# dallison/subspace

Hardware: AMD Instinct MI355X
Metric: GiB/s CRC32 over batched payloads (device-resident); % of HBM3E read peak (higher is better)
Workload: dtype u8

## Files before the change

subspace_amd/_lib.py:

```python
from __future__ import annotations

import ctypes
import os
from pathlib import Path

_HERE = Path(__file__).resolve().parent
LIB_PATH = _HERE / "libsubspace_crc.so"
if os.environ.get("SUBSPACE_CRC_PROBE_LIB"):
    LIB_PATH = Path(os.environ["SUBSPACE_CRC_PROBE_LIB"])
DEV_LIB_PATH = _HERE / "libsubspace_crc_dev.so"
if os.environ.get("SUBSPACE_CRC_PROBE_DEV_LIB"):
    DEV_LIB_PATH = Path(os.environ["SUBSPACE_CRC_PROBE_DEV_LIB"])

EXPORTED_SYMBOLS = (
    "SubspaceCRC32",
    "SubspaceCRC32C",
    "subspace_crc_version",
    "subspace_crc_last_error",
    "subspace_crc_ctx_create",
    "subspace_crc_ctx_create_poly",
    "subspace_crc_ctx_destroy",
    "subspace_crc_ctx_check",
    "subspace_crc_ctx_reserve",
    "subspace_crc32_batch_uniform",
# ... 78 lines not shown
    u32, u64, vp, i32 = ctypes.c_uint32, ctypes.c_uint64, ctypes.c_void_p, ctypes.c_int
    lib.subspace_crc_testutil_fill_uniform.restype = i32
    lib.subspace_crc_testutil_fill_uniform.argtypes = [vp, u64, u64, u64, u64, u64, u64, vp]
    lib.subspace_crc_testutil_fill_ragged.restype = i32
    lib.subspace_crc_testutil_fill_ragged.argtypes = [vp, vp, vp, u64, u64, u64, u64, vp]
    lib.subspace_crc_testutil_tune.restype = i32
    lib.subspace_crc_testutil_tune.argtypes = [vp, i32, i32, i32]
    lib.subspace_crc_testutil_set.restype = i32
    lib.subspace_crc_testutil_set.argtypes = [vp, ctypes.c_char_p, i32]
    lib.subspace_crc_testutil_stream_read.restype = i32
    lib.subspace_crc_testutil_stream_read.argtypes = [vp, u64, vp, vp]
    lib.subspace_crc_testutil_stream_read_lds.restype = i32
    lib.subspace_crc_testutil_stream_read_lds.argtypes = [vp, u64, vp, ctypes.c_uint32, vp]
    lib.subspace_crc_testutil_uniform_alias.restype = i32
    lib.subspace_crc_testutil_uniform_alias.argtypes = [vp, vp, u64, vp, vp]
    lib.subspace_crc_testutil_probe.restype = i32
    lib.subspace_crc_testutil_probe.argtypes = [vp, vp]
    lib.subspace_crc_testutil_probe_waves.restype = u64
    lib.subspace_crc_testutil_probe_waves.argtypes = [vp, u64]
    lib.subspace_crc_testutil_slot_list_read.restype = i32
    lib.subspace_crc_testutil_slot_list_read.argtypes = [vp, u64, u32, u64, u32, vp, u64, vp]
    lib.subspace_crc_testutil_tile_list_read.restype = i32
    lib.subspace_crc_testutil_tile_list_read.argtypes = [vp, u64, vp, u64, vp]
    lib.subspace_crc_testutil_fault_words.restype = i32
    lib.subspace_crc_testutil_fault_words.argtypes = [vp, vp, vp]
    lib.subspace_crc_testutil_call_gen.restype = u32
    lib.subspace_crc_testutil_call_gen.argtypes = [vp]
    _dev = lib
    return lib


def last_error() -> str:
    msg = load().subspace_crc_last_error()
    return msg.decode() if msg else ""
```

subspace_amd/csrc/capi.hip:

```cpp
#include <hip/hip_runtime.h>

#include <algorithm>
#include <cstdarg>
#include <cstdio>
#include <cstring>
#include <mutex>
#include <vector>

#include "../../include/subspace_crc.h"
#include "crc_device.h"
#include "crc_math.h"
#include "ctx.h"

namespace subspace_amd {

template <int WG, bool SLOT, bool PROBE>
__global__ void crc32_uniform4k_kernel(const uint8_t*, u64, u64, const u32*, const u32*, u32, u32, u32*, int, u32*,
                                       SlotArgs);

struct TileDesc;
struct TileDesc8;
__global__ void crc32_ragged_count_desc_kernel(const u64*, u32, const u64*, u32, u64, u32, u32, u64*, u32*, u32*,
                                               u64*, u32*, u64, TileDesc8*, u32*, FaultRef);
__global__ void crc32_ragged_count_desc16_kernel(const u64*, u32, const u64*, u32, u64, u32, u32, u64*, u32*, u32*,
                                                 u64*, u32*, u64, TileDesc*, u32*, FaultRef);
__global__ void crc32_ragged_count_scan_kernel(const u64*, u32, const u64*, u32, u64, u32, u32, u64*, u32*, u32*,
                                               u64*, u32*, u32*, FaultRef);
__global__ void tile_segment_scan_kernel(const u32*, u32, u32, u32, const u64*, u64, u32*, u32*);
__global__ void segment_prefix_kernel(u32*, u64, u32, u32, const u64*, u64, u64*, u32*, FaultRef);
__global__ void crc32_ragged_desc_kernel(const u64*, u32, const u64*, u32, const u64*, u64, u64, TileDesc*, u32*,
                                         u64*, u64, u32*, FaultRef);
template <int WG>
__global__ void crc32_ragged_kernel(const uint8_t*, const u64*, u32, const u64*, u32, const u64*, u64,
                                    const TileDesc*, const u32*, const u32*, const u32*, HeadSeeds, u32*, u32*, u32,
                                    u64*, u64, u32*, FaultRef);
__global__ void crc32_ragged_final_kernel(const u64*, const u64*, u32, const u64*, u32, u64, const u32*, const u32*,
                                          u32, u32, u32*, const u32*, u32, u32*, u64*, u64, u32*, FaultRef);
__global__ void crc32_slot_finish_kernel(const u64*, uint8_t*, u64, const u64*, u64, u64, u64, int, int, u32,
                                         const u32*, const u32*, const u32*, u32*, u32*, u32*);
__global__ void slot_payload_offsets_kernel(u64, u64, u64, u64*, const u64*, u64, u64*);
__global__ void uniform_offsets_kernel(u64 stride, u64 length, u64 count, u64* offsets, u64* lengths);
template <int WG>
__global__ void crc32_long_kernel(const uint8_t*, u64, u32, u32, const u32*, const u32*, u32, u32, u32*, u32);
__global__ void crc32_long_final_kernel(const u32*, const u32*, u32, u32, u32, u32, u32*, u64*, u64, u32*);
template <int WG, bool SLOT, bool PROBE, int G>
__global__ void crc32_small_kernel(const u32*, const u32*, SmallArgs);

}

using namespace subspace_amd;

namespace {

thread_local char g_err[512] = "";

int fail(int code, const char* fmt, ...) {
  va_list ap;
  va_start(ap, fmt);
  vsnprintf(g_err, sizeof(g_err), fmt, ap);
  va_end(ap);
  return code;
}
int hip_fail(hipError_t e, const char* what) {
  return fail(SUBSPACE_CRC_EHIP, "%s: %s", what, hipGetErrorString(e));
}
#define HIP_TRY(call)                                   \
  do {                                                  \
    hipError_t e_ = (call);                             \
    if (e_ != hipSuccess) return hip_fail(e_, #call);   \
// ... 54 lines not shown
        c->ws_stream = c->ws_call_stream;
        c->ws_recorded = true;
      }
      c->ws_waited = false;
    }
  }
  CallScope(const CallScope&) = delete;
  CallScope& operator=(const CallScope&) = delete;
};

int use_workspace(subspace_crc_ctx* c, hipStream_t st) {
  if (c->ws_waited) return SUBSPACE_CRC_OK;
  if (!c->ws_done) HIP_TRY(hipEventCreateWithFlags(&c->ws_done, hipEventDisableTiming));
  if (c->ws_recorded && c->ws_stream != st && !capturing(st)) HIP_TRY(hipStreamWaitEvent(st, c->ws_done, 0));
  c->ws_waited = true;
  c->ws_call_stream = st;
  return SUBSPACE_CRC_OK;
}

const char* fault_text(u32 f) {
  if (f & kFaultTicket) return "a look-back scan ticket was beyond its grid (stale scan state)";
  if (f & kFaultLookbackSpin) return "a look-back scan predecessor never published (stale scan state)";
  if (f & kFaultSlotRing) return "a fused slot kernel finishing wave never received a payload CRC";
  return "unknown fault";
}

int fault_status(subspace_crc_ctx* c, hipStream_t st) {
  u32 f = 0;
  HIP_TRY(hipMemcpyAsync(&f, c->d_fault, sizeof(u32), hipMemcpyDeviceToHost, st));
  HIP_TRY(hipStreamSynchronize(st));
  if (f == 0) return SUBSPACE_CRC_OK;
  if (f & kFaultSlotRing) {
    HIP_TRY(hipDeviceSynchronize());
    HIP_TRY(hipMemcpy(&f, c->d_fault, sizeof(u32), hipMemcpyDeviceToHost));
    HIP_TRY(hipMemset(c->d_slot_counter, 0, kSlotCounters * kCountWords * sizeof(u64)));
    HIP_TRY(hipDeviceSynchronize());
  }
  HIP_TRY(hipMemsetAsync(c->d_fault, 0, sizeof(u32), st));
  HIP_TRY(hipStreamSynchronize(st));
  c->scan_dirty = true;
  return fail(SUBSPACE_CRC_EFAULT, "device fault 0x%x: %s; the results of the calls since the last check are not valid",
              f, fault_text(f));
}

struct TileGeom {
  u64 nw, nkmax, nwb, nseg, nblk;
};
TileGeom tile_geom(const subspace_crc_ctx* c, u64 tiles) {
  TileGeom g;
  g.nw = (u64)c->num_cus * (kRaggedWG / 64);
  g.nkmax = ceil_div(tiles ? tiles : 1, g.nw);
  g.nwb = ceil_div(g.nw, 64);
  g.nseg = g.nkmax * g.nwb;
  g.nblk = ceil_div(g.nkmax, 64) * g.nwb;
  return g;
// ... 209 lines not shown
        default: crc32_small_kernel<512, true, false, 32><<<blocks, 512, lds, st>>>(c->d_tab, c->d_laneops, a);
#undef SMALL_SLOT_CASE
      }
    }
  } else {
    a.zero_word = c->zero_word;
    c->zero_word = nullptr;
    switch (g) {
#define SMALL_CASE(G) \
  case G: crc32_small_kernel<512, false, false, G><<<blocks, 512, lds, st>>>(c->d_tab, c->d_laneops, a); break;
      SMALL_CASE(1) SMALL_CASE(2) SMALL_CASE(4) SMALL_CASE(8) SMALL_CASE(16)
      default: crc32_small_kernel<512, false, false, 32><<<blocks, 512, lds, st>>>(c->d_tab, c->d_laneops, a);
#undef SMALL_CASE
    }
  }
  HIP_TRY(hipGetLastError());
  return SUBSPACE_CRC_OK;
}

bool small_slot_fused(int32_t checksum_size, int32_t metadata_size) {
  return (u32)checksum_size <= kSlotFusedMaxMeta && (u32)metadata_size <= kSlotFusedMaxMeta;
}

int ensure_slot_ws(subspace_crc_ctx* c, u64 count) {
  if (count <= c->s_capacity) return SUBSPACE_CRC_OK;
  (void)hipFree(c->d_crc0);
  (void)hipFree(c->d_soff);
  (void)hipFree(c->d_slen);
  c->d_crc0 = nullptr;
  c->d_soff = nullptr;
  c->d_slen = nullptr;
  c->s_capacity = 0;
  HIP_TRY(hipMalloc(&c->d_crc0, count * sizeof(u32)));
  HIP_TRY(hipMalloc(&c->d_soff, count * sizeof(u64)));
  HIP_TRY(hipMalloc(&c->d_slen, count * sizeof(u64)));
  c->s_capacity = count;
  return SUBSPACE_CRC_OK;
}

int check_slot_args(int32_t checksum_size, int32_t metadata_size, uint32_t mode) {
  if (mode != SUBSPACE_CRC_SLOT_CALCULATE && mode != SUBSPACE_CRC_SLOT_VERIFY)
    return fail(SUBSPACE_CRC_EINVAL, "unknown slot mode %u", mode);
  if (checksum_size < 4) return fail(SUBSPACE_CRC_EINVAL, "checksum_size %d < 4", checksum_size);
  if (metadata_size < 0) return fail(SUBSPACE_CRC_EINVAL, "metadata_size %d < 0", metadata_size);
  return SUBSPACE_CRC_OK;
}
// ... 111 lines not shown
  if (e == hipSuccess) e = hipMemset(c->d_slot_counter, 0, kSlotCounters * kCountWords * sizeof(u64));
  if (e == hipSuccess) e = hipMalloc(&c->d_fault, 4 * sizeof(u32));
  if (e == hipSuccess) e = hipMemset(c->d_fault, 0, 4 * sizeof(u32));
  if (e == hipSuccess) e = hipEventCreateWithFlags(&c->ws_done, hipEventDisableTiming);
  if (e == hipSuccess) e = hipDeviceSynchronize();
  if (e == hipSuccess)
    e = hipFuncSetAttribute((const void*)crc32_ragged_kernel<kRaggedWG>, hipFuncAttributeMaxDynamicSharedMemorySize,
                            (int)ragged_lds_bytes());
  if (e == hipSuccess)
    e = hipFuncSetAttribute((const void*)crc32_long_kernel<kRaggedWG>, hipFuncAttributeMaxDynamicSharedMemorySize,
                            (int)ragged_lds_bytes());
  {
    const void* small_fns[] = {
        (const void*)crc32_small_kernel<512, false, false, 1>,  (const void*)crc32_small_kernel<512, true, false, 1>,
        (const void*)crc32_small_kernel<512, false, false, 2>,  (const void*)crc32_small_kernel<512, true, false, 2>,
        (const void*)crc32_small_kernel<512, false, false, 4>,  (const void*)crc32_small_kernel<512, true, false, 4>,
        (const void*)crc32_small_kernel<512, false, false, 8>,  (const void*)crc32_small_kernel<512, true, false, 8>,
        (const void*)crc32_small_kernel<512, false, false, 16>, (const void*)crc32_small_kernel<512, true, false, 16>,
        (const void*)crc32_small_kernel<512, false, false, 32>, (const void*)crc32_small_kernel<512, true, false, 32>};
    for (const void* f : small_fns)
      if (e == hipSuccess)
        e = hipFuncSetAttribute(f, hipFuncAttributeMaxDynamicSharedMemorySize, (int)small_lds_bytes() + 16);
  }
  if (e != hipSuccess) {
    subspace_crc_ctx_destroy(c);
    return hip_fail(e, "context setup");
  }
  *out = c;
  return SUBSPACE_CRC_OK;
}

void subspace_crc_ctx_destroy(subspace_crc_ctx* c) {
  if (!c) return;
  if (c->ws_done && c->ws_recorded) (void)hipEventSynchronize(c->ws_done);
  if (c->hcompute) (void)hipStreamSynchronize(c->hcompute);
  for (auto& h : c->hstage) {
    if (h.stream) (void)hipStreamSynchronize(h.stream);
    if (h.copied) (void)hipEventDestroy(h.copied);
    (void)hipFree(h.dbuf);
    (void)hipFree(h.dsizes);
    (void)hipFree(h.dres);
    (void)hipFree(h.derr);
    (void)hipHostFree(h.hres);
    (void)hipHostFree(h.herr);
    if (h.done) (void)hipEventDestroy(h.done);
    if (h.stream) (void)hipStreamDestroy(h.stream);
// ... 147 lines not shown

int subspace_crc32_slots(subspace_crc_ctx* c, const subspace_crc_slot* dev_slots, uint64_t count,
                         uint64_t max_message_size, int32_t checksum_size, int32_t metadata_size, uint32_t mode,
                         uint32_t* dev_status, uint32_t* dev_error_count, void* stream) {
  g_err[0] = 0;
  if (!c) return fail(SUBSPACE_CRC_EINVAL, "ctx is null");
  CallScope scope(c);
  int rc = check_slot_args(checksum_size, metadata_size, mode);
  if (rc) return rc;
  hipStream_t st = (hipStream_t)stream;
  if (count == 0) {
    if (dev_error_count) HIP_TRY(hipMemsetAsync(dev_error_count, 0, sizeof(u32), st));
    return SUBSPACE_CRC_OK;
  }
  if (!dev_slots) return fail(SUBSPACE_CRC_EINVAL, "null device pointer");
  if (count >= (1ull << 32)) return fail(SUBSPACE_CRC_EINVAL, "count %llu exceeds 2^32-1", (unsigned long long)count);
  HIP_TRY(hipSetDevice(c->device));
  const u64* rec = reinterpret_cast<const u64*>(dev_slots);
  const bool small = max_message_size <= kSmallMaxExt && c->small_path;
  if (small && small_slot_fused(checksum_size, metadata_size)) {
    const SmallSlot ss{rec, 3, 0, ~0ull, mode, checksum_size, metadata_size, dev_status, nullptr, dev_error_count};
    return small_run(c, nullptr, rec + 1, 3, rec + 2, 3, count, 0u, 0u, nullptr, st, &ss, small_lanes(max_message_size));
  }
  rc = use_workspace(c, st);
  if (rc) return rc;
  rc = ensure_slot_ws(c, count);
  if (rc) return rc;
  want_zeroed(c, dev_error_count);
  if (small) {
    rc = small_run(c, nullptr, rec + 1, 3, rec + 2, 3, count, 0u, 0u, c->d_crc0, st, nullptr,
                   small_lanes(max_message_size));
  } else {
    const u64 cap = count * ((max_message_size + 15 + 8191) / 8192) + 1;
    rc = ragged_run(c, nullptr, cap, rec + 1, 3, rec + 2, 3, count, 0u, 0u, c->d_crc0, st, 0);
  }
  const bool zeroed = was_zeroed(c, dev_error_count);
  if (rc) return rc;
  return slot_finish(c, rec, nullptr, 0, nullptr, 0, count, ~0ull, checksum_size, metadata_size, mode, dev_status,
                     dev_error_count, st, nullptr, zeroed);
}

}

namespace {

int slots_strided_impl(subspace_crc_ctx* c, void* dev_buffer, uint64_t slot_stride, uint64_t count,
// ... 340 lines not shown
```

subspace_amd/csrc/crc_combine.hip:

```cpp
#include "crc_desc.h"

namespace subspace_amd {

constexpr int kScanThreads = 256;
constexpr int kScanItems = (int)(kScanTile / kScanThreads);
static_assert(kScanTile % kScanThreads == 0, "segment-prefix scan: whole items per thread");
constexpr int kCountItems = (int)(kCountTile / kScanThreads);
static_assert(kCountTile % kScanThreads == 0, "tile-count scan: whole items per thread");
constexpr u64 kFlagAggregate = 1, kFlagInclusive = 2;

struct SumOp {
  using T = u64;
  static __device__ __forceinline__ T identity() { return 0; }
  static __device__ __forceinline__ T op(T a, T b) { return a + b; }
  static __device__ __forceinline__ u64 pack(u64 flag, T v) { return (flag << 62) | v; }
  static __device__ __forceinline__ u64 flag(u64 s) { return s >> 62; }
  static __device__ __forceinline__ T value(u64 s) { return s & ((1ull << 62) - 1); }
};

struct XorOp {
  using T = u32;
  static __device__ __forceinline__ T identity() { return 0; }
  static __device__ __forceinline__ T op(T a, T b) { return a ^ b; }
  static __device__ __forceinline__ u64 pack(u64 flag, T v) { return (flag << 32) | v; }
// ... 146 lines not shown
  for (int j = 0; j < kCountItems; j++) {
    const u64 i = base + (u64)(j * kScanThreads + tid);
    if (i <= count) tile_base[i] = sx[j * kScanThreads + tid];
  }
}

constexpr int kFusedThreads = 1024;
constexpr int kFusedItems = (int)(kCountTile / kFusedThreads);
static_assert(kCountTile % kFusedThreads == 0, "fused scan: whole items per thread");
template <bool WIDE>
__device__ __forceinline__ void count_desc_body(const u64* __restrict__ offsets, u32 ostride,
                                                const u64* __restrict__ lengths, u32 lstride, u64 count, u32 init,
                                                u32 final_xor, u64* __restrict__ tile_base, u32* __restrict__ out,
                                                u32* __restrict__ zero_word, u64* __restrict__ status,
                                                u32* __restrict__ ticket, u64 capacity, void* __restrict__ desc,
                                                u32* __restrict__ overflow, FaultRef fault) {
  __shared__ u64 sx[kCountTile];
  __shared__ u32 sw[WIDE ? 1 : kFusedThreads / 64][kDesc8WaveWords][64];
  bool stale;
  const u64 tile = scan_ticket(ticket, fault, &stale, true);
  if (stale) return;
  const u64 base = tile * kCountTile;
  const int tid = threadIdx.x;
  if (WIDE && tid == 0) overflow[1] = 1u;
  u64 so[kFusedItems], L[kFusedItems], nt[kFusedItems];
  bool bad = false;
#pragma unroll
  for (int j = 0; j < kFusedItems; j++) {
    const u64 i = base + (u64)(j * kFusedThreads + tid);
    so[j] = L[j] = nt[j] = 0;
    if (i < count) {
      so[j] = offsets[i * ostride];
      L[j] = lengths[i * lstride];
      nt[j] = msg_tiles(so[j], L[j]);
      out[i] = nt[j] == 0 ? init ^ final_xor : 0u;
      if (!WIDE && nt[j] &&
          ((((so[j] & ~(u64)15) + ((nt[j] - 1) << 13)) >> kDesc8StartBits) | ((nt[j] - 1) >> kDesc8AfterBits)))
        bad = true;
    } else if (i == count && zero_word) {
      *zero_word = 0u;
    }
    sx[j * kFusedThreads + tid] = nt[j];
  }
  if (bad) overflow[2] = 1u;
  __syncthreads();
  u64 x[kFusedItems];
#pragma unroll
// ... 122 lines not shown
```

subspace_amd/csrc/crc_device.h:

```cpp
#pragma once
#include <hip/hip_runtime.h>
#include <stdint.h>

namespace subspace_amd {

using u32 = uint32_t;
using u64 = uint64_t;
using i64 = int64_t;
using u32x4 = __attribute__((ext_vector_type(4))) unsigned int;
using u32x2 = __attribute__((ext_vector_type(2))) unsigned int;

constexpr u32 kLdsTables = 0;
constexpr u32 kLdsOps = 128u * 1024u;

constexpr int kLaneOpWords = 8 * 16 * 32;
constexpr int kUniSlotOpZ4096 = kLaneOpWords * 4 / 512;
constexpr int kUniSlotOpZ64 = kUniSlotOpZ4096 + 1;
constexpr int kUniOpSlots = kUniSlotOpZ64 + 4;
constexpr int kUniOpSlotsOneChain = kUniSlotOpZ4096 + 1;
constexpr u32 kUniRing = kLdsOps + kUniOpSlots * 512u;
constexpr int uni_ring_results(int waves) { return kUniRing + (u32)waves * 1024u <= 160u * 1024u ? 256 : 128; }
constexpr size_t uniform_lds_bytes(int waves) { return kUniRing + (size_t)waves * 4u * uni_ring_results(waves); }
static_assert(uniform_lds_bytes(16) <= 160u * 1024u && uniform_lds_bytes(8) <= 160u * 1024u,
              "uniform kernel LDS exceeds 160 KiB");
// ... 2 lines not shown
constexpr int kSlotFinishers = 4;
constexpr u32 kSlotRingBytesPerWave = 2u * 8u * kSlotRingRounds;
constexpr u32 uniform_slot_mism_word(int waves) { return kUniSlotRing + (u32)waves * kSlotRingBytesPerWave; }
constexpr size_t uniform_slot_lds_bytes(int waves) { return uniform_slot_mism_word(waves) + 16u; }
static_assert(uniform_slot_lds_bytes(8) <= 160u * 1024u, "slot kernel LDS exceeds 160 KiB");

struct SlotArgs {
  u64 prefix_size;
  u32 mode;
  u32* status;
  u32* crc_out;
  u32* error_count;
  u64* counter;
  u64* probe;
  u32* fault;
  u32 checksum_size;
  u32 metadata_size;
};
constexpr u32 kSlotFusedMaxMeta = 64;

constexpr u32 kFaultLookbackSpin = 1u;
constexpr u32 kFaultTicket = 2u;
constexpr u32 kFaultSlotRing = 4u;
__device__ __forceinline__ void raise_fault(u32* fault, u32 bit) {
  if (fault) __hip_atomic_fetch_or(fault, bit, __ATOMIC_RELAXED, __HIP_MEMORY_SCOPE_AGENT);
}
struct FaultRef {
  u32* word;
  u32 gen;
};
__device__ __forceinline__ void raise_scan_fault(FaultRef f, u32 bit) {
  if (f.word) {
    __hip_atomic_fetch_or(f.word, bit, __ATOMIC_RELAXED, __HIP_MEMORY_SCOPE_AGENT);
    __hip_atomic_store(f.word + 1, f.gen, __ATOMIC_RELAXED, __HIP_MEMORY_SCOPE_AGENT);
  }
}
__device__ __forceinline__ bool scan_faulted(FaultRef f) {
  return f.word && f.word[1] == f.gen;
}
constexpr u32 kSpinBound = 1u << 20;
constexpr int kProbeWords = 8;

constexpr int kNumTileOps = 21;
constexpr int kRagOpZ4096 = kLaneOpWords * 4 / 512;
constexpr int kRagOpZTile = kRagOpZ4096 + 1;
constexpr int kRagZ64Words = kLaneOpWords + (1 + kNumTileOps) * 128;
constexpr int kRagLdsOpWords = kRagZ64Words + 512;
constexpr int kRagHighOps = kRagLdsOpWords;
constexpr int kNumInvOps = 13;
constexpr int kRagInvOps = kRagHighOps + (31 - kNumTileOps) * 128;
constexpr int kRagNibInvOps = kRagInvOps + kNumInvOps * 128;
constexpr int kNumNibInvOps = 45;
constexpr int kRagOpWords = kRagNibInvOps + kNumNibInvOps * 128;
constexpr size_t ragged_lds_bytes() { return kLdsOps + (size_t)kRagLdsOpWords * 4u; }
static_assert(ragged_lds_bytes() <= 160u * 1024u, "ragged kernel LDS exceeds 160 KiB");

constexpr int kSmallOpInv = kUniOpSlots;
constexpr int kSmallInvOps = 12;
constexpr int kSmallOpSlots = kSmallOpInv + kSmallInvOps;
constexpr int kSmallOpZC = kSmallOpSlots;
constexpr int kSmallLaneOpSlots = kSmallOpZC + 5;
constexpr u32 kSmallMaxExt = 4096;
constexpr u32 kSmallRing = kLdsOps + (u32)(kSmallOpSlots + 1) * 512u;
constexpr u32 kSmallRingTiles = 32;
constexpr u32 kSmallRingBytesPerWave = kSmallRingTiles * 2u * 8u;
constexpr u32 kRp2Entries = 256;
constexpr u32 kRp2MaxTiles = kRp2Entries * 32u / 64u;
constexpr u32 kRp2EntS = kSmallRing;
constexpr u32 kRp2EntM = kRp2EntS + 8u * kRp2Entries;
constexpr u32 kRp2Ring = kRp2EntM + 4u * kRp2Entries;
constexpr u32 kRp2Starts = kRp2Ring + 8u * kRp2Entries;
constexpr u32 kRp2First = kRp2Starts + 8u * kRp2MaxTiles;
constexpr u32 kRp2Misc = kRp2First + 4u * kRp2MaxTiles;
constexpr u32 kRp2Counts = kRp2Misc + 176u;
constexpr u32 kRp2Bytes = kRp2Counts + 128u - kSmallRing;
constexpr u32 kSmallShared = 8u * kSmallRingBytesPerWave > kRp2Bytes ? 8u * kSmallRingBytesPerWave : kRp2Bytes;
constexpr size_t small_lds_bytes() { return kSmallRing + kSmallShared; }
static_assert(small_lds_bytes() + 16u <= 160u * 1024u, "small-message kernel LDS (+ mismatch word) exceeds 160 KiB");
// ... 248 lines not shown
  if constexpr (SUBSPACE_ISSUE_PRIO > 0) __builtin_amdgcn_s_setprio(0);
}

__device__ __forceinline__ u64 tilecrc_index(u64 w, u64 k, u32 nwb) {
  return ((((k >> 6) * nwb + (w >> 6)) << 6 | (w & 63)) << 6) | (k & 63);
}
__device__ __forceinline__ u64 local_index(u64 w, u64 k, u32 nwb) {
  return ((((k >> 6) * nwb + (w >> 6)) << 6 | (k & 63)) << 6) | (w & 63);
}
__device__ __forceinline__ u32 tile_prefix(const u32* __restrict__ local, const u32* __restrict__ segx, u32 nw,
                                           u32 nwb, u64 tau) {
  const u32 t = (u32)tau, k = t / nw, w = t - k * nw;
  return segx[(u64)k * nwb + (w >> 6)] ^ local[local_index(w, k, nwb)];
}

__device__ __forceinline__ void reset_scan_state(u64* status, u64 nwords, u32* ticket) {
  const u64 g = (u64)blockIdx.x * blockDim.x + threadIdx.x, stride = (u64)gridDim.x * blockDim.x;
  for (u64 i = g; i < nwords; i += stride) __hip_atomic_store(&status[i], 0ull, __ATOMIC_RELAXED, __HIP_MEMORY_SCOPE_AGENT);
  if (g == 0) __hip_atomic_store(ticket, 0u, __ATOMIC_RELAXED, __HIP_MEMORY_SCOPE_AGENT);
}

#ifndef SUBSPACE_COUNT_GROUPS
#define SUBSPACE_COUNT_GROUPS 1
#endif
constexpr u32 kCountGroups = SUBSPACE_COUNT_GROUPS;
constexpr u32 kCountWords = 16;
__device__ __forceinline__ void add_call_mismatches(u64* counter, u32 n, u32* error_count) {
  if constexpr (kCountGroups == 1) {
    const u64 old = atomicAdd(reinterpret_cast<unsigned long long*>(counter), (1ull << 32) | (u64)n);
    if ((u32)(old >> 32) == gridDim.x - 1u) {
      *error_count = (u32)old + n;
      __hip_atomic_store(counter, 0ull, __ATOMIC_RELAXED, __HIP_MEMORY_SCOPE_AGENT);
    }
    return;
  }
  const u32 G = gridDim.x, g = blockIdx.x % kCountGroups;
  const u32 ng = (G - g + kCountGroups - 1u) / kCountGroups;
  const u64 old = atomicAdd(reinterpret_cast<unsigned long long*>(counter + 1 + g), (1ull << 32) | (u64)n);
  if ((u32)(old >> 32) == ng - 1u) {
    const u32 tot = (u32)old + n;
    __hip_atomic_store(counter + 1 + g, 0ull, __ATOMIC_RELAXED, __HIP_MEMORY_SCOPE_AGENT);
    const u32 groups = G < kCountGroups ? G : kCountGroups;
    const u64 o2 = atomicAdd(reinterpret_cast<unsigned long long*>(counter), (1ull << 32) | (u64)tot);
    if ((u32)(o2 >> 32) == groups - 1u) {
      *error_count = (u32)o2 + tot;
      __hip_atomic_store(counter, 0ull, __ATOMIC_RELAXED, __HIP_MEMORY_SCOPE_AGENT);
    }
  }
}
// ... 9 lines not shown
```

subspace_amd/csrc/ctx.h:

```cpp
#pragma once
#include <hip/hip_runtime.h>

#include <mutex>

#include "../../include/subspace_crc.h"
#include "crc_device.h"
#include "crc_math.h"

namespace subspace_amd {

struct DevHooks {
  u64* probe = nullptr;
  hipError_t (*uniform)(bool slot, unsigned blocks, hipStream_t st, const uint8_t* base, u64 stride, u64 count,
                        const u32* tab, const u32* ops, u32 init, u32 final_xor, u32* out, u32* zero_word,
                        SlotArgs sa) = nullptr;
  hipError_t (*small_slot)(unsigned blocks, size_t lds, hipStream_t st, const u32* tab, const u32* ops,
                           const SmallArgs& a) = nullptr;
};

constexpr uint32_t kCtxMagic = 0x43524353u;

}

struct subspace_crc_ctx {
// ... 34 lines not shown
    hipEvent_t copied = nullptr;
    hipEvent_t done = nullptr;
    uint8_t* dbuf = nullptr;
    subspace_amd::u64* dsizes = nullptr;
    subspace_amd::u32* dres = nullptr;
    subspace_amd::u32* derr = nullptr;
    subspace_amd::u32* hres = nullptr;
    subspace_amd::u32* herr = nullptr;
  } hstage[2];
  subspace_amd::u64 h_bytes = 0, h_slots = 0;
  subspace_crc_slot* l_hrec = nullptr;
  subspace_crc_slot* l_drec = nullptr;
  subspace_amd::u32* l_dstatus = nullptr;
  subspace_amd::u32* l_hstatus = nullptr;
  subspace_amd::u64 l_capacity = 0;
  subspace_amd::u32* d_crc0 = nullptr;
  subspace_amd::u64* d_soff = nullptr;
  subspace_amd::u64* d_slen = nullptr;
  subspace_amd::u64 s_capacity = 0;
  subspace_amd::u64* d_slot_counter = nullptr;
  subspace_amd::u32 slot_counter_next = 0;
  bool fused_slots = true;
  bool small_path = true;
  subspace_amd::DevHooks dev;
  subspace_amd::u32* d_fault = nullptr;
  subspace_amd::u32 call_gen = 0;
  std::recursive_mutex mu;
  int depth = 0;
  hipEvent_t ws_done = nullptr;
  hipStream_t ws_stream = nullptr;
  bool ws_recorded = false;
  bool ws_waited = false;
  hipStream_t ws_call_stream = nullptr;
};
```

subspace_amd/csrc/devtools.hip:

```cpp
#define SUBSPACE_DEV_TU 1
#include "crc_small.hip"
#include "crc_uniform.hip"
#include "ctx.h"

#include <algorithm>
#include <cstring>

namespace subspace_amd {
template __global__ void crc32_small_kernel<512, true, true, 32>(const u32*, const u32*, SmallArgs);
template __global__ void crc32_uniform4k_kernel<512, false, true>(const uint8_t*, u64, u64, const u32*, const u32*, u32,
                                                                  u32, u32*, int, u32*, SlotArgs);
template __global__ void crc32_uniform4k_kernel<512, true, true>(const uint8_t*, u64, u64, const u32*, const u32*, u32,
                                                                 u32, u32*, int, u32*, SlotArgs);
template __global__ void crc32_uniform4k_kernel<512, false, false>(const uint8_t*, u64, u64, const u32*, const u32*,
                                                                   u32, u32, u32*, int, u32*, SlotArgs);
}

using namespace subspace_amd;

namespace {

bool ctx_ok(const subspace_crc_ctx* c) {
  return c && c->magic == kCtxMagic && c->layout_bytes == (uint32_t)sizeof(subspace_crc_ctx);
}
// ... 39 lines not shown
  }();
  return e;
}

}

extern "C" {

int subspace_crc_testutil_set(subspace_crc_ctx* c, const char* key, int value) {
  if (!ctx_ok(c) || !key) return SUBSPACE_CRC_EINVAL;
  std::lock_guard<std::recursive_mutex> lk(c->mu);
  if (!std::strcmp(key, "stale_ticket")) {
    if (!c->d_scan_state) return SUBSPACE_CRC_EINVAL;
    const u32 v = (u32)value;
    if (hipSetDevice(c->device) != hipSuccess || hipDeviceSynchronize() != hipSuccess ||
        hipMemcpy(c->d_scan_state, &v, sizeof(u32), hipMemcpyHostToDevice) != hipSuccess)
      return SUBSPACE_CRC_EHIP;
    return SUBSPACE_CRC_OK;
  }
  bool* knob = !std::strcmp(key, "long_path")     ? &c->long_path
               : !std::strcmp(key, "fused_slots") ? &c->fused_slots
               : !std::strcmp(key, "fused_prep")  ? &c->fused_prep
               : !std::strcmp(key, "small_path")  ? &c->small_path
                                                  : nullptr;
  if (!knob) return SUBSPACE_CRC_EINVAL;
  *knob = value != 0;
  return SUBSPACE_CRC_OK;
}

int subspace_crc_testutil_tune(subspace_crc_ctx* c, int uniform_wg, int uniform_blocks, int uniform_order) {
  if (!ctx_ok(c) || uniform_wg != 512 || uniform_order < 0 || uniform_order > 3 || uniform_blocks < 0)
    return SUBSPACE_CRC_EINVAL;
  std::lock_guard<std::recursive_mutex> lk(c->mu);
  c->uniform_blocks = uniform_blocks;
  c->uniform_order = uniform_order;
  return SUBSPACE_CRC_OK;
}

int subspace_crc_testutil_probe(subspace_crc_ctx* c, void* dev_words) {
  if (!ctx_ok(c)) return SUBSPACE_CRC_EINVAL;
  std::lock_guard<std::recursive_mutex> lk(c->mu);
  if (dev_words) {
    if (hipSetDevice(c->device) != hipSuccess || set_lds_attributes() != hipSuccess) return SUBSPACE_CRC_EHIP;
    c->dev.uniform = uniform_probe;
    c->dev.small_slot = small_slot_probe;
  }
// ... 35 lines not shown
```

subspace_amd/csrc/testutil.hip:

```cpp
#include <hip/hip_runtime.h>
#include <stdint.h>

#include "crc_device.h"

namespace {

__device__ __forceinline__ uint64_t splitmix64(uint64_t x) {
  uint64_t z = x + 0x9E3779B97F4A7C15ull;
  z = (z ^ (z >> 30)) * 0xBF58476D1CE4E5B9ull;
  z = (z ^ (z >> 27)) * 0x94D049BB133111EBull;
  return z ^ (z >> 31);
}

__global__ void synth_fill_kernel(uint8_t* __restrict__ base, const uint64_t* __restrict__ offsets,
                                  const uint64_t* __restrict__ lengths, uint64_t stride, uint64_t length,
                                  uint64_t count, uint64_t first_id, uint64_t id_stride, uint64_t seed) {
  for (uint64_t m = blockIdx.x; m < count; m += gridDim.x) {
    const uint64_t off = offsets ? offsets[m] : m * stride;
    const uint64_t len = lengths ? lengths[m] : length;
    const uint64_t id = first_id + m * id_stride;
    const uint64_t key = seed ^ (id << 32);
    uint8_t* dst = base + off;
    const uint64_t units = (len + 7) >> 3;
    const bool aligned8 = (off & 7) == 0;
// ... 219 lines not shown
  };
  u64 a0, a1;
  u32 n0, n1;
  desc(0, a0, n0);
  u32x4 A[8], B[8];
  load(A, a0, n0);
  u64 k = 0;
  for (; k + 1 < nk; k += 2) {
    desc(k + 1, a1, n1);
    drain_before_issue();
    load(B, a1, n1);
    fold(A);
    desc(k + 2, a0, n0);
    drain_before_issue();
    load(A, a0, n0);
    fold(B);
  }
  drain_before_issue();
  if (k < nk) fold(A);
  if (acc == 0x12345678u && ntiles == 1) lds_unused3[threadIdx.x] = acc;
  out[blockIdx.x * 512 + threadIdx.x] = acc;
}

}

extern "C" {

int subspace_crc_testutil_tile_list_read(const void* dev_tiles, uint64_t ntiles, unsigned* dev_out,
                                         uint64_t out_words, void* stream) {
  if (!dev_tiles || !dev_out || ntiles == 0) return -1;
  int dev = 0, cus = 0;
  if (hipGetDevice(&dev) != hipSuccess || hipDeviceGetAttribute(&cus, hipDeviceAttributeMultiprocessorCount, dev) != hipSuccess)
    return -2;
  if (out_words < (uint64_t)cus * 512) return -1;
  const size_t ldsb = subspace_amd::ragged_lds_bytes();
  if (hipFuncSetAttribute((const void*)tile_list_read_kernel, hipFuncAttributeMaxDynamicSharedMemorySize, (int)ldsb) !=
      hipSuccess)
    return -2;
  tile_list_read_kernel<<<(unsigned)cus, 512, ldsb, (hipStream_t)stream>>>(static_cast<const uint64_t*>(dev_tiles),
                                                                             ntiles, dev_out);
  return hipGetLastError() == hipSuccess ? 0 : -2;
}

int subspace_crc_testutil_slot_list_read(const void* dev_records, uint64_t count, uint32_t mode, uint64_t stride,
                                         uint32_t lds, unsigned* dev_out, uint64_t out_words, void* stream) {
  if (!dev_records || !dev_out || count == 0 || mode > 6) return -1;
  int dev = 0, cus = 0;
  if (hipGetDevice(&dev) != hipSuccess || hipDeviceGetAttribute(&cus, hipDeviceAttributeMultiprocessorCount, dev) != hipSuccess)
    return -2;
// ... 69 lines not shown
```

subspace_amd/gpu.py:

```python
from __future__ import annotations

import ctypes

from . import _lib

FINALIZE = 0x1
POLY_IEEE = 0xEDB88320
POLY_CASTAGNOLI = 0x82F63B78

SLOT_CALCULATE = 0
SLOT_VERIFY = 1
SLOT_OK, SLOT_MISMATCH, SLOT_UNCHECKED, SLOT_OVERSIZE = 0, 1, 2, 4
EFAULT = -5


class CrcError(RuntimeError):
    def __init__(self, msg: str, code: int = 0):
        super().__init__(msg)
        self.code = code


def _check(rc: int, what: str) -> None:
    if rc != 0:
        raise CrcError(f"{what} failed ({rc}): {_lib.last_error()}", rc)
# ... 145 lines not shown
def fill_uniform(buf, stride: int, length: int, count: int, *, seed: int, first_id: int = 0, id_stride: int = 1,
                 stream=None) -> None:
    _check(_lib.load_dev().subspace_crc_testutil_fill_uniform(
        _ptr(buf), stride, length, count, first_id, id_stride, seed, _stream_ptr(stream)), "fill_uniform")


def fill_ragged(buf, offsets, lengths, *, seed: int, first_id: int = 0, id_stride: int = 1, stream=None) -> None:
    _check(_lib.load_dev().subspace_crc_testutil_fill_ragged(
        _ptr(buf), _ptr(offsets), _ptr(lengths), int(offsets.numel()), first_id, id_stride, seed,
        _stream_ptr(stream)), "fill_ragged")


def slot_list_read(records, count: int, out, mode: int = 4, stride: int = 0, lds: bool = True, stream=None) -> None:
    _check(_lib.load_dev().subspace_crc_testutil_slot_list_read(
        _ptr(records), int(count), int(mode), int(stride), 1 if lds else 0, _ptr(out), int(out.numel()),
        _stream_ptr(stream)), "slot_list_read")


def tile_list_read(tiles, out, stream=None) -> None:
    _check(_lib.load_dev().subspace_crc_testutil_tile_list_read(
        _ptr(tiles), int(tiles.shape[0]), _ptr(out), int(out.numel()), _stream_ptr(stream)), "tile_list_read")


def stream_read(buf, out, stream=None) -> None:
    if int(out.numel()) < 256 * 512:
        raise ValueError("out needs 131072 words")
    _check(_lib.load_dev().subspace_crc_testutil_stream_read(
        _ptr(buf), int(buf.numel() * buf.element_size()), _ptr(out), _stream_ptr(stream)), "stream_read")
```

Measured before the change: 5584.

## Add fused single-pass medium-message slot-list CRC kernel with per-wave message streaming

Adds a new kernel for slot lists whose messages fall between the small-path limit and 32 KiB. Each wave streams whole messages in 8 KiB tiles with double-buffered loads, drawn from workgroup-level chunk tickets. It then folds the header/metadata CRC and writes or verifies the checksum in batches of 64, replacing the multi-kernel workspace path. This targets launch and workspace overheads and intermediate global traffic. The cost is a new spin-wait chunk ring with a fault path, plus a memory-read test utility.

```diff
diff --git a/subspace_amd/_lib.py b/subspace_amd/_lib.py
--- a/subspace_amd/_lib.py
+++ b/subspace_amd/_lib.py
@@ -124,6 +124,9 @@
     lib.subspace_crc_testutil_slot_list_read.argtypes = [vp, u64, u32, u64, u32, vp, u64, vp]
     lib.subspace_crc_testutil_tile_list_read.restype = i32
     lib.subspace_crc_testutil_tile_list_read.argtypes = [vp, u64, vp, u64, vp]
+    if hasattr(lib, "subspace_crc_testutil_msg_list_read"):
+        lib.subspace_crc_testutil_msg_list_read.restype = i32
+        lib.subspace_crc_testutil_msg_list_read.argtypes = [vp, u64, vp, u64, vp]
     lib.subspace_crc_testutil_fault_words.restype = i32
     lib.subspace_crc_testutil_fault_words.argtypes = [vp, vp, vp]
     lib.subspace_crc_testutil_call_gen.restype = u32
diff --git a/subspace_amd/csrc/capi.hip b/subspace_amd/csrc/capi.hip
--- a/subspace_amd/csrc/capi.hip
+++ b/subspace_amd/csrc/capi.hip
@@ -45,6 +45,8 @@
 __global__ void crc32_long_final_kernel(const u32*, const u32*, u32, u32, u32, u32, u32*, u64*, u64, u32*);
 template <int WG, bool SLOT, bool PROBE, int G>
 __global__ void crc32_small_kernel(const u32*, const u32*, SmallArgs);
+template <int WG>
+__global__ void crc32_medium_slots_kernel(const u32*, const u32*, MediumArgs);
 
 }
 
@@ -145,6 +147,7 @@
   if (f & kFaultTicket) return "a look-back scan ticket was beyond its grid (stale scan state)";
   if (f & kFaultLookbackSpin) return "a look-back scan predecessor never published (stale scan state)";
   if (f & kFaultSlotRing) return "a fused slot kernel finishing wave never received a payload CRC";
+  if (f & kFaultMediumChunk) return "a medium slot kernel wave never received its workgroup's next chunk";
   return "unknown fault";
 }
 
@@ -153,7 +156,7 @@
   HIP_TRY(hipMemcpyAsync(&f, c->d_fault, sizeof(u32), hipMemcpyDeviceToHost, st));
   HIP_TRY(hipStreamSynchronize(st));
   if (f == 0) return SUBSPACE_CRC_OK;
-  if (f & kFaultSlotRing) {
+  if (f & (kFaultSlotRing | kFaultMediumChunk)) {
     HIP_TRY(hipDeviceSynchronize());
     HIP_TRY(hipMemcpy(&f, c->d_fault, sizeof(u32), hipMemcpyDeviceToHost));
     HIP_TRY(hipMemset(c->d_slot_counter, 0, kSlotCounters * kCountWords * sizeof(u64)));
@@ -409,6 +412,28 @@
   return (u32)checksum_size <= kSlotFusedMaxMeta && (u32)metadata_size <= kSlotFusedMaxMeta;
 }
 
+bool medium_slot_list(const subspace_crc_ctx* c, u64 max_message_size, int32_t checksum_size, int32_t metadata_size) {
+  return c->medium_path && max_message_size > kSmallMaxExt && max_message_size <= kMedMaxMessage &&
+         small_slot_fused(checksum_size, metadata_size);
+}
+int medium_run(subspace_crc_ctx* c, const u64* rec, u64 count, int32_t checksum_size, int32_t metadata_size, u32 mode,
+               u32* status, u32* error_count, hipStream_t st) {
+  MediumArgs a{};
+  a.rec = rec;
+  a.count = count;
+  a.mode = mode;
+  a.checksum_size = (u32)checksum_size;
+  a.metadata_size = (u32)metadata_size;
+  a.status = status;
+  a.error_count = error_count;
+  a.counter = c->d_slot_counter + kCountWords * (c->slot_counter_next++ % kSlotCounters);
+  a.fault = c->d_fault;
+  const unsigned blocks = (unsigned)grid_for(c, ceil_div(count, kMedChunk), 1);
+  crc32_medium_slots_kernel<512><<<blocks, 512, medium_lds_bytes(), st>>>(c->d_tab, c->d_rops, a);
+  HIP_TRY(hipGetLastError());
+  return SUBSPACE_CRC_OK;
+}
+
 int ensure_slot_ws(subspace_crc_ctx* c, u64 count) {
   if (count <= c->s_capacity) return SUBSPACE_CRC_OK;
   (void)hipFree(c->d_crc0);
@@ -566,6 +591,9 @@
       if (e == hipSuccess)
         e = hipFuncSetAttribute(f, hipFuncAttributeMaxDynamicSharedMemorySize, (int)small_lds_bytes() + 16);
   }
+  if (e == hipSuccess)
+    e = hipFuncSetAttribute((const void*)crc32_medium_slots_kernel<512>, hipFuncAttributeMaxDynamicSharedMemorySize,
+                            (int)medium_lds_bytes());
   if (e != hipSuccess) {
     subspace_crc_ctx_destroy(c);
     return hip_fail(e, "context setup");
@@ -759,6 +787,8 @@
     const SmallSlot ss{rec, 3, 0, ~0ull, mode, checksum_size, metadata_size, dev_status, nullptr, dev_error_count};
     return small_run(c, nullptr, rec + 1, 3, rec + 2, 3, count, 0u, 0u, nullptr, st, &ss, small_lanes(max_message_size));
   }
+  if (medium_slot_list(c, max_message_size, checksum_size, metadata_size))
+    return medium_run(c, rec, count, checksum_size, metadata_size, mode, dev_status, dev_error_count, st);
   rc = use_workspace(c, st);
   if (rc) return rc;
   rc = ensure_slot_ws(c, count);
diff --git a/subspace_amd/csrc/crc_combine.hip b/subspace_amd/csrc/crc_combine.hip
--- a/subspace_amd/csrc/crc_combine.hip
+++ b/subspace_amd/csrc/crc_combine.hip
@@ -192,7 +192,7 @@
   if (stale) return;
   const u64 base = tile * kCountTile;
   const int tid = threadIdx.x;
-  if (WIDE && tid == 0) overflow[1] = 1u;
+  if (tid == 0) overflow[1] = WIDE ? 1u : 0u;
   u64 so[kFusedItems], L[kFusedItems], nt[kFusedItems];
   bool bad = false;
 #pragma unroll
diff --git a/subspace_amd/csrc/crc_device.h b/subspace_amd/csrc/crc_device.h
--- a/subspace_amd/csrc/crc_device.h
+++ b/subspace_amd/csrc/crc_device.h
@@ -48,6 +48,7 @@
 constexpr u32 kFaultLookbackSpin = 1u;
 constexpr u32 kFaultTicket = 2u;
 constexpr u32 kFaultSlotRing = 4u;
+constexpr u32 kFaultMediumChunk = 8u;
 __device__ __forceinline__ void raise_fault(u32* fault, u32 bit) {
   if (fault) __hip_atomic_fetch_or(fault, bit, __ATOMIC_RELAXED, __HIP_MEMORY_SCOPE_AGENT);
 }
@@ -80,6 +81,28 @@
 constexpr int kRagOpWords = kRagNibInvOps + kNumNibInvOps * 128;
 constexpr size_t ragged_lds_bytes() { return kLdsOps + (size_t)kRagLdsOpWords * 4u; }
 static_assert(ragged_lds_bytes() <= 160u * 1024u, "ragged kernel LDS exceeds 160 KiB");
+
+constexpr int kMedTileOps = 3;
+constexpr int kMedFillSlots = kRagOpZTile + kMedTileOps;
+constexpr int kMedOpZ64 = kMedFillSlots;
+constexpr int kMedOpInv = kMedOpZ64 + 4;
+constexpr int kMedOpSlots = kMedOpInv + kNumInvOps;
+constexpr u32 kMedCtl = kLdsOps + 512u * (u32)kMedOpSlots;
+constexpr u32 kMedRing = 16;
+constexpr size_t medium_lds_bytes() { return kMedCtl + 64u + 8u * kMedRing; }
+static_assert(medium_lds_bytes() <= 160u * 1024u, "medium slot kernel LDS exceeds 160 KiB");
+constexpr u32 kMedChunk = 16;
+constexpr u32 kMedMaxMessage = 32768;
+
+struct MediumArgs {
+  const u64* rec;
+  u64 count;
+  u32 mode, checksum_size, metadata_size;
+  u32* status;
+  u32* error_count;
+  u64* counter;
+  u32* fault;
+};
 
 constexpr int kSmallOpInv = kUniOpSlots;
 constexpr int kSmallInvOps = 12;
@@ -374,9 +397,13 @@
 
 #ifndef SUBSPACE_COUNT_GROUPS
 #define SUBSPACE_COUNT_GROUPS 1
+#elif !defined(SUBSPACE_AB_BUILD)
+#error "SUBSPACE_COUNT_GROUPS is a timing-only knob: build with tools/ab_lib.sh (SUBSPACE_AB_BUILD)"
 #endif
 constexpr u32 kCountGroups = SUBSPACE_COUNT_GROUPS;
 constexpr u32 kCountWords = 16;
+static_assert(kCountGroups >= 1 && kCountGroups + 1 <= kCountWords, "the group words overrun the counter entry");
+static_assert(kCountGroups + 2 <= kCountWords, "the group words reach the chunk ticket");
 __device__ __forceinline__ void add_call_mismatches(u64* counter, u32 n, u32* error_count) {
   if constexpr (kCountGroups == 1) {
     const u64 old = atomicAdd(reinterpret_cast<unsigned long long*>(counter), (1ull << 32) | (u64)n);
diff --git a/subspace_amd/csrc/crc_medium.hip b/subspace_amd/csrc/crc_medium.hip
--- /dev/null
+++ b/subspace_amd/csrc/crc_medium.hip
@@ -0,0 +1,325 @@
+#include "crc_device.h"
+
+namespace subspace_amd {
+
+namespace {
+constexpr u32 kMedHasChecksum = 4u;
+constexpr u32 kMedNone = 0xFFFFFFFFu;
+
+typedef __attribute__((address_space(1))) u64 glb_u64_t;
+typedef __attribute__((address_space(1))) u32 glb_u32_t;
+
+__device__ __forceinline__ u64 readlane64(u64 v, int l) {
+  const u32 lo = (u32)__builtin_amdgcn_readlane((int)(u32)v, l);
+  const u32 hi = (u32)__builtin_amdgcn_readlane((int)(u32)(v >> 32), l);
+  return ((u64)hi << 32) | lo;
+}
+
+struct MedMsg {
+  u64 s0;
+  u64 ext;
+  u64 pfx;
+  u64 len;
+  u64 nt;
+  u32 mis;
+  u32 idx;
+};
+
+template <int WG>
+struct MedOpFill {
+  static constexpr int kWords = (4 + kNumInvOps) * 128;
+  static constexpr int kIters = (kWords + WG - 1) / WG;
+  u32 v[kIters];
+  __device__ __forceinline__ void load(const u32* __restrict__ gops) {
+#pragma unroll
+    for (int i = 0; i < kIters; i++) {
+      const int t = min((int)threadIdx.x + i * WG, kWords - 1);
+      v[i] = gops[t < 512 ? kRagZ64Words + t : kRagInvOps + (t - 512)];
+    }
+  }
+  __device__ __forceinline__ void store(u32 sbase) const {
+#pragma unroll
+    for (int i = 0; i < kIters; i++) {
+      const int t = (int)threadIdx.x + i * WG;
+      if (t < kWords) lds_st(sbase + kLdsOps + 512u * (u32)kMedOpZ64 + 4u * (u32)t, v[i]);
+    }
+#pragma unroll
+    for (int i = 0; i < kIters; i++) asm volatile("" ::"v"(v[i]));
+  }
+};
+}
+
+template <int WG>
+__global__ __launch_bounds__(WG) void crc32_medium_slots_kernel(const u32* __restrict__ gtab,
+                                                                const u32* __restrict__ gops, MediumArgs a) {
+  extern __shared__ __attribute__((aligned(16))) u32 smem[];
+  const u32 sbase = (u32)(uintptr_t)smem;
+  const int lane = threadIdx.x & 63;
+  const u32 lc0 = sbase + ((u32)(lane & 31) << 2);
+  const u32 lc1 = lc0 + 0x10000u;
+  const u32 z64 = sbase + kLdsOps + 512u * (u32)kMedOpZ64 + 4u * (u32)(lane & 3);
+  const u32 lop = sbase + kLdsOps + 4u * (u32)(31 - (lane & 31));
+  const u32 ctl = sbase + kMedCtl, ring = ctl + 64u;
+  const bool calc = a.mode == 0u;
+  u32* const gticket = reinterpret_cast<u32*>(a.counter + (kCountWords - 1));
+  const u32 G = rfl(gridDim.x);
+
+  if (threadIdx.x == 0) {
+    lds_st(ctl, 0u);
+    lds_st(ctl + 8u, 0u);
+  }
+  if (threadIdx.x < kMedRing)
+    lds_st64(ring + 8u * threadIdx.x, threadIdx.x == 0 ? (u64)blockIdx.x : ~0ull);
+  __syncthreads();
+
+  LdsFill<WG, kMedFillSlots> fill;
+  fill.load(gtab, gops);
+  MedOpFill<WG> xfill;
+  xfill.load(gops);
+
+  auto draw = [&]() __attribute__((always_inline)) -> u32 {
+    u32 t = 0;
+    if (lane == 0)
+      t = __hip_atomic_fetch_add(reinterpret_cast<lds_u32_t*>((uintptr_t)ctl), 1u, __ATOMIC_RELAXED,
+                                 __HIP_MEMORY_SCOPE_WORKGROUP);
+    t = rfl(t);
+    const u32 q = t / kMedChunk, r = t % kMedChunk;
+    if (r == 0u) {
+      u32 g = 0;
+      if (lane == 0) g = atomicAdd(gticket, 1u);
+      if (lane == 0) lds_st64(ring + 8u * ((q + 1u) % kMedRing), (u64)(G + g) | ((u64)(q + 1u) << 32));
+    }
+    u64 e = 0;
+    u32 spins = 0;
+    for (;;) {
+      const u64 v = lds_ld64(ring + 8u * (q % kMedRing));
+      e = rfl64((u32)v, (u32)(v >> 32));
+      if ((u32)(e >> 32) == q) break;
+      if (++spins > kSpinBound) {
+        if (lane == 0) raise_fault(a.fault, kFaultMediumChunk);
+        return kMedNone;
+      }
+      __builtin_amdgcn_s_sleep(1);
+    }
+    const u64 idx = (u64)(u32)e * kMedChunk + r;
+    return idx < a.count ? (u32)idx : kMedNone;
+  };
+  auto rec_load = [&](u32 idx) __attribute__((always_inline)) -> u64 {
+    const u64* p = a.rec + 3ull * (idx == kMedNone ? 0u : idx) + (u32)min(lane, 2);
+    const u64 v = *p;
+    asm volatile("" ::"v"(p));
+    return v;
+  };
+  auto unpack = [&](u64 R, u32 idx) __attribute__((always_inline)) -> MedMsg {
+    MedMsg m;
+    m.pfx = readlane64(R, 0);
+    const u64 s = readlane64(R, 1);
+    m.len = idx == kMedNone ? 0ull : readlane64(R, 2);
+    m.idx = idx;
+    m.mis = (u32)s & 15u;
+    m.s0 = s & ~(u64)15;
+    m.ext = m.len ? m.len + m.mis : 0ull;
+    const u64 nt = (m.ext + 8191u) >> 13;
+    m.nt = nt ? nt : 1ull;
+    return m;
+  };
+  const u32 vo = (u32)lane * 128u;
+  auto load_line = [&](const MedMsg& m, u64 j, u32x4 (&L)[8]) __attribute__((always_inline)) {
+    const u64 rest = m.ext - (j << 13);
+    const u32 len = rest < 8192u ? (u32)rest : 8192u;
+    const u32 nrec = (len + 15u) & ~15u;
+    const auto r = __builtin_amdgcn_make_buffer_rsrc(reinterpret_cast<uint8_t*>(m.s0 + (j << 13)), (short)0,
+                                                     (int)nrec, kBufferRsrcFlags);
+#pragma unroll
+    for (int b = 0; b < 8; b++) L[b] = __builtin_amdgcn_raw_buffer_load_b128(r, vo + 16u * b, 0, 0);
+    __builtin_amdgcn_sched_barrier(0);
+  };
+
+  auto tile_value = [&](const u32x4 (&cur)[8], const MedMsg& m, u64 j) __attribute__((always_inline)) -> u32 {
+    const u64 rest = m.ext - (j << 13);
+    const u32 len = rest < 8192u ? (u32)rest : 8192u;
+    u32x4 d[8];
+#pragma unroll
+    for (int b = 0; b < 8; b++) d[b] = cur[b];
+    const bool head = j == 0 && m.mis != 0u, tail = len < 8192u && (len & 15u) != 0u;
+    if (head || tail) {
+      const int v0 = (int)len - 128 * lane;
+      const u32 hi = v0 <= 0 ? 0u : (v0 >= 128 ? 128u : (u32)v0);
+      const u32 lo = (head && lane == 0) ? m.mis : 0u;
+      keep_bytes(d, lo, hi);
+    }
+    const u32 crc = line_crc32_2chain(d, 0u, lc0, lc1, z64);
+    u32 v = lane_shift(lop, crc);
+    v ^= (u32)__builtin_amdgcn_update_dpp(0, (int)v, 0x111, 0xF, 0xF, false);
+    v ^= (u32)__builtin_amdgcn_update_dpp(0, (int)v, 0x112, 0xF, 0xF, false);
+    v ^= (u32)__builtin_amdgcn_update_dpp(0, (int)v, 0x114, 0xF, 0xF, false);
+    v ^= (u32)__builtin_amdgcn_update_dpp(0, (int)v, 0x118, 0xF, 0xF, false);
+    v ^= (u32)__builtin_amdgcn_update_dpp(0, (int)v, 0x142, 0xA, 0xF, false);
+    const u32 h0 = (u32)__builtin_amdgcn_readlane((int)v, 31), h1 = (u32)__builtin_amdgcn_readlane((int)v, 63);
+    return opmul(sbase, kRagOpZ4096, h0) ^ h1;
+  };
+
+  auto inv_bits = [&](u32 x, u32 bits, int nb) __attribute__((always_inline)) {
+    for (int b = 0; b < nb && __any(bits != 0u); b++) {
+      if (__any((bits & 1u) != 0u)) {
+        const u32 xm = opmul(sbase, kMedOpInv + b, x);
+        x = (bits & 1u) ? xm : x;
+      }
+      bits >>= 1;
+    }
+    return x;
+  };
+
+  u64 PFX = 0, PLEN = 0;
+  u32 PMIS = 0, PIDX = 0, PVAL = 0;
+  u32 mism = 0;
+
+  auto flush = [&](u32 n) __attribute__((always_inline)) {
+    const bool valid = (u32)lane < n;
+    const u64 pa = valid ? PFX : readlane64(PFX, 0);
+    const u64 L = valid ? PLEN : 0ull;
+    const u32 mis = valid ? PMIS : 0u;
+    u32 w[14];
+    {
+      const glb_u64_t* q = reinterpret_cast<const glb_u64_t*>(pa);
+#pragma unroll
+      for (int i = 0; i < 7; i++) {
+        const u64 x = q[i];
+        w[2 * i] = (u32)x;
+        w[2 * i + 1] = (u32)(x >> 32);
+      }
+      asm volatile("" ::"v"(q));
+    }
+    const bool has = (w[8] & kMedHasChecksum) != 0u;
+    const u32 F = calc ? (w[8] | kMedHasChecksum) : w[8];
+    const u32 S = w[12];
+    w[8] = F;
+    u32 h = 0xFFFFFFFFu;
+#pragma unroll
+    for (int i = 1; i < 12; i++) h = step4(h ^ w[i], lc0, lc1);
+    if (a.metadata_size) {
+      constexpr u32 kW = kSlotFusedMaxMeta / 4 + 2;
+      const u32 o1 = 48u + a.checksum_size, sh = o1 & 3u, ms = a.metadata_size;
+      const u32 nwords = (sh + ms + 3u) >> 2;
+      const glb_u32_t* p1 = reinterpret_cast<const glb_u32_t*>(pa + (o1 & ~3u));
+      u32 W1[kW];
+#pragma unroll
+      for (u32 j = 0; j < kW; j++) W1[j] = p1[min(j, nwords - 1u)];
+      u32 tl = 0;
+#pragma unroll
+      for (u32 j = 0; j + 1 < kW; j++) {
+        const u32 x = __builtin_amdgcn_alignbyte(W1[j + 1], W1[j], sh);
+        if (j < (ms >> 2)) h = step4(h ^ x, lc0, lc1);
+        if (j == (ms >> 2)) tl = x;
+      }
+      for (u32 b = 0; b < (ms & 3u); b++) h = step1(h, (tl >> (8u * b)) & 0xFFu, lc1);
+    }
+    const u64 ext = L ? L + mis : 0ull;
+    const u64 nt = (ext + 8191u) >> 13;
+    u32 x = inv_bits(h, L ? mis : 0u, 4);
+    {
+      u64 rem = nt;
+      int bit = 0;
+      for (; bit < kMedTileOps && __any(rem != 0ull); bit++) {
+        const u32 xm = opmul(sbase, kRagOpZTile + bit, x);
+        x = (rem & 1u) ? xm : x;
+        rem >>= 1;
+      }
+      for (; bit < 31 && __any(rem != 0ull); bit++) {
+        const u32* op = gops + (bit < kNumTileOps ? kLaneOpWords + 128 * (1 + bit)
+                                                  : kRagHighOps + 128 * (bit - kNumTileOps));
+        const u32 xm = opmul_global(op, x);
+        x = (rem & 1u) ? xm : x;
+        rem >>= 1;
+      }
+    }
+    x ^= PVAL;
+    x = inv_bits(x, (u32)((nt << 13) - ext), kNumInvOps);
+    const u32 crc = ~x;
+    glb_u32_t* const pw = reinterpret_cast<glb_u32_t*>(pa);
+    bool bad = false;
+    if (valid) {
+      if (calc) {
+        if (!has) pw[8] = F;
+        pw[12] = crc;
+        if (a.status) a.status[PIDX] = 0u;
+      } else if (!has) {
+        if (a.status) a.status[PIDX] = 2u;
+      } else {
+        bad = S != crc;
+        if (a.status) a.status[PIDX] = bad ? 1u : 0u;
+      }
+    }
+    mism += (u32)__builtin_popcountll(__ballot(bad));
+  };
+
+  const u32 idx0 = draw();
+  const u64 R0 = rec_load(idx0);
+  MedMsg C = unpack(R0, idx0);
+  u32 idxN = idx0 == kMedNone ? kMedNone : draw();
+  u64 RN = rec_load(idxN);
+  u32x4 A[8], B[8];
+  load_line(C, 0, A);
+  fill.store(sbase);
+  xfill.store(sbase);
+  __syncthreads();
+
+  u64 j = 0;
+  u32 acc = 0, np = 0;
+  auto step = [&](const u32x4 (&cur)[8], u32x4 (&nxt)[8]) __attribute__((always_inline)) {
+    issue_prio_hi();
+    drain_before_issue();
+    const bool last = j + 1 >= C.nt;
+    MedMsg X = C;
+    u64 jx = j + 1;
+    if (last) {
+      X = unpack(RN, idxN);
+      jx = 0;
+      if (idxN != kMedNone) idxN = draw();
+    }
+    RN = rec_load(idxN);
+    load_line(X, jx, nxt);
+    issue_prio_lo();
+    const u32 t = tile_value(cur, C, j);
+    acc = j ? opmul(sbase, kRagOpZTile, acc) ^ t : t;
+    if (last && C.idx != kMedNone) {
+      const bool mine = lane == (int)np;
+      PFX = mine ? C.pfx : PFX;
+      PLEN = mine ? C.len : PLEN;
+      PMIS = mine ? C.mis : PMIS;
+      PIDX = mine ? C.idx : PIDX;
+      PVAL = mine ? acc : PVAL;
+      np++;
+      asm volatile("" : "+s"(np));
+      if (np == 64u) {
+        flush(64u);
+        np = 0;
+      }
+    }
+    C = X;
+    j = jx;
+  };
+  while (C.idx != kMedNone) {
+    step(A, B);
+    step(B, A);
+  }
+  if (np) flush(np);
+
+  if (lane == 0 && mism)
+    __hip_atomic_fetch_add(reinterpret_cast<lds_u32_t*>((uintptr_t)(ctl + 8u)), mism, __ATOMIC_RELAXED,
+                           __HIP_MEMORY_SCOPE_WORKGROUP);
+  __syncthreads();
+  if (threadIdx.x == 0) {
+    const u32 n = lds_ld_volatile(ctl + 8u);
+    const u64 old = atomicAdd(reinterpret_cast<unsigned long long*>(a.counter), (1ull << 32) | (u64)n);
+    if ((u32)(old >> 32) == G - 1u) {
+      if (a.error_count) *a.error_count = (u32)old + n;
+      __hip_atomic_store(gticket, 0u, __ATOMIC_RELAXED, __HIP_MEMORY_SCOPE_AGENT);
+      __hip_atomic_store(a.counter, 0ull, __ATOMIC_RELAXED, __HIP_MEMORY_SCOPE_AGENT);
+    }
+  }
+}
+
+template __global__ void crc32_medium_slots_kernel<512>(const u32*, const u32*, MediumArgs);
+
+}
diff --git a/subspace_amd/csrc/ctx.h b/subspace_amd/csrc/ctx.h
--- a/subspace_amd/csrc/ctx.h
+++ b/subspace_amd/csrc/ctx.h
@@ -80,6 +80,7 @@
   subspace_amd::u32 slot_counter_next = 0;
   bool fused_slots = true;
   bool small_path = true;
+  bool medium_path = true;
   subspace_amd::DevHooks dev;
   subspace_amd::u32* d_fault = nullptr;
   subspace_amd::u32 call_gen = 0;
diff --git a/subspace_amd/csrc/devtools.hip b/subspace_amd/csrc/devtools.hip
--- a/subspace_amd/csrc/devtools.hip
+++ b/subspace_amd/csrc/devtools.hip
@@ -85,6 +85,7 @@
                : !std::strcmp(key, "fused_slots") ? &c->fused_slots
                : !std::strcmp(key, "fused_prep")  ? &c->fused_prep
                : !std::strcmp(key, "small_path")  ? &c->small_path
+               : !std::strcmp(key, "medium_path") ? &c->medium_path
                                                   : nullptr;
   if (!knob) return SUBSPACE_CRC_EINVAL;
   *knob = value != 0;
diff --git a/subspace_amd/csrc/testutil.hip b/subspace_amd/csrc/testutil.hip
--- a/subspace_amd/csrc/testutil.hip
+++ b/subspace_amd/csrc/testutil.hip
@@ -265,9 +265,96 @@
   out[blockIdx.x * 512 + threadIdx.x] = acc;
 }
 
+__global__ __launch_bounds__(512) void msg_list_read_kernel(const uint64_t* __restrict__ rec, uint64_t count,
+                                                            unsigned* __restrict__ out) {
+  using namespace subspace_amd;
+  extern __shared__ unsigned lds_unused4[];
+  const int lane = threadIdx.x & 63;
+  const u64 w = front_slot(blockIdx.x, gridDim.x, rfl(threadIdx.x >> 6));
+  const u64 nw = (u64)gridDim.x * 8;
+  auto rec_load = [&](u64 m) {
+    const uint64_t* p = rec + 3 * (m < count ? m : count - 1) + (u32)min(lane, 2);
+    const u64 v = *p;
+    asm volatile("" ::"v"(p));
+    return v;
+  };
+  auto lane64 = [&](u64 v, int l) {
+    return ((u64)(u32)__builtin_amdgcn_readlane((int)(u32)(v >> 32), l) << 32) |
+           (u32)__builtin_amdgcn_readlane((int)(u32)v, l);
+  };
+  struct Msg {
+    u64 s0, ext, nt;
+  };
+  auto unpack = [&](u64 R, bool live) {
+    const u64 s = lane64(R, 1), L = live ? lane64(R, 2) : 0;
+    Msg m;
+    m.s0 = s & ~(u64)15;
+    m.ext = L ? L + (s & 15) : 0;
+    m.nt = m.ext ? (m.ext + 8191) >> 13 : 1;
+    return m;
+  };
+  auto load = [&](u32x4 (&L)[8], const Msg& m, u64 j) {
+    const u64 rest = m.ext - (j << 13);
+    const u32 n = ((rest < 8192 ? (u32)rest : 8192u) + 15u) & ~15u;
+    const auto r = __builtin_amdgcn_make_buffer_rsrc(reinterpret_cast<void*>(m.s0 + (j << 13)), (short)0, (int)n,
+                                                     kBufferRsrcFlags);
+#pragma unroll
+    for (int b = 0; b < 8; b++) L[b] = __builtin_amdgcn_raw_buffer_load_b128(r, (u32)lane * 128u + 16u * b, 0, 0);
+    __builtin_amdgcn_sched_barrier(0);
+  };
+  unsigned acc = 0;
+  auto fold = [&](const u32x4 (&D)[8]) {
+#pragma unroll
+    for (int b = 0; b < 8; b++) acc ^= D[b].x ^ D[b].y ^ D[b].z ^ D[b].w;
+  };
+  u64 m = w, j = 0;
+  Msg C = unpack(rec_load(m), m < count);
+  u64 RN = rec_load(m + nw);
+  u32x4 A[8], B[8];
+  load(A, C, 0);
+  auto step = [&](const u32x4 (&cur)[8], u32x4 (&nxt)[8]) {
+    drain_before_issue();
+    Msg X = C;
+    u64 jx = j + 1;
+    if (jx >= C.nt) {
+      m += nw;
+      X = unpack(RN, m < count);
+      jx = 0;
+    }
+    RN = rec_load(m + nw);
+    load(nxt, X, jx);
+    fold(cur);
+    C = X;
+    j = jx;
+  };
+  while (m < count) {
+    step(A, B);
+    step(B, A);
+  }
+  drain_before_issue();
+  if (acc == 0x12345678u && count == 1) lds_unused4[threadIdx.x] = acc;
+  out[blockIdx.x * 512 + threadIdx.x] = acc;
+}
+
 }
 
 extern "C" {
+
+int subspace_crc_testutil_msg_list_read(const void* dev_records, uint64_t count, unsigned* dev_out,
+                                        uint64_t out_words, void* stream) {
+  if (!dev_records || !dev_out || count == 0) return -1;
+  int dev = 0, cus = 0;
+  if (hipGetDevice(&dev) != hipSuccess || hipDeviceGetAttribute(&cus, hipDeviceAttributeMultiprocessorCount, dev) != hipSuccess)
+    return -2;
+  if (out_words < (uint64_t)cus * 512) return -1;
+  const size_t ldsb = subspace_amd::medium_lds_bytes();
+  if (hipFuncSetAttribute((const void*)msg_list_read_kernel, hipFuncAttributeMaxDynamicSharedMemorySize, (int)ldsb) !=
+      hipSuccess)
+    return -2;
+  msg_list_read_kernel<<<(unsigned)cus, 512, ldsb, (hipStream_t)stream>>>(static_cast<const uint64_t*>(dev_records),
+                                                                           count, dev_out);
+  return hipGetLastError() == hipSuccess ? 0 : -2;
+}
 
 int subspace_crc_testutil_tile_list_read(const void* dev_tiles, uint64_t ntiles, unsigned* dev_out,
                                          uint64_t out_words, void* stream) {
diff --git a/subspace_amd/gpu.py b/subspace_amd/gpu.py
--- a/subspace_amd/gpu.py
+++ b/subspace_amd/gpu.py
@@ -191,6 +191,11 @@
         _ptr(tiles), int(tiles.shape[0]), _ptr(out), int(out.numel()), _stream_ptr(stream)), "tile_list_read")
 
 
+def msg_list_read(records, out, stream=None) -> None:
+    _check(_lib.load_dev().subspace_crc_testutil_msg_list_read(
+        _ptr(records), int(records.shape[0]), _ptr(out), int(out.numel()), _stream_ptr(stream)), "msg_list_read")
+
+
 def stream_read(buf, out, stream=None) -> None:
     if int(out.numel()) < 256 * 512:
         raise ValueError("out needs 131072 words")
```

Result: slower. 5511 (-1.3%).
